# bkram/fmtuner-sdr

Hardware: AMD Instinct MI355X
Metric: IQ MS/s demodulated per GPU (2.4 MS/s FM channels, stereo+RDS) at 1/2/4/8 MI355X (higher is better)
Workload: dtype f32 (FIR operands f16 hi+lo, f32 accumulate)

## Files before the change

fmtuner-sdr_amd/csrc/fmx_kernels.hip:

```cpp
#include <hip/hip_ext.h>
#include <hip/hip_fp16.h>
#include <hip/hip_runtime.h>

#include <cstddef>
#include <type_traits>

#include "fmx_internal.h"
#include "fmx_math.h"
#include "fmx_synth.h"


namespace fmx {

#define FE_T 768
#define FE_HALO_IQ 120
#define AU_T 768
#define AU_HALO 120
#define AU_RHALO 32
#define AU_MAXOUT 256

static constexpr float kPiF = 3.14159265358979323846f;

#define FMX_CONST __attribute__((address_space(4)))
template <typename T> __device__ __forceinline__ const FMX_CONST T *cptr(const T *p) {
// ... 525 lines not shown
        fe_decimate<M, TPP>(inq, Q, D->dec_poly, tid, ai, aq);
        int myclip = 0;
#pragma unroll
        for (int r = 0; r < 3; ++r) {
          const int j = 3 * tid + r;
          if (j < cnt) {
            const float yr = ai[r] * D->dec_scale;
            const float yi = aq[r] * D->dec_scale;
            if (fabsf(yr) >= 0.995f || fabsf(yi) >= 0.995f) myclip++;
            xin[FE_HALO_IQ + j] = make_float2(yr, yi);
            if (a.bb_out) {
              float *o = a.bb_out + (size_t)c * a.bb_stride + 2 * (size_t)(n0 + j);
              o[0] = yr;
              o[1] = yi;
            }
          }
        }
        if (myclip) atomicAdd(&sh->clip, myclip);
        __syncthreads();
      }
    } else if (a.in_mode == FE_IN_CF) {
      int myclip = 0;
      for (int j = tid; j < cnt; j += 256) {
        const float *p = a.in_f + (size_t)c * a.in_stride + 2 * (size_t)(n0 + j);
        const float xr = p[0], xi = p[1];
        if (fabsf(xr) >= 0.995f || fabsf(xi) >= 0.995f) myclip++;
        xin[FE_HALO_IQ + j] = make_float2(xr, xi);
      }
      if (myclip) atomicAdd(&sh->clip, myclip);
    } else if (a.in_mode == FE_IN_U8_DIRECT) {
      int myclip = 0;
      const uint8_t *p = a.iq + (size_t)c * a.iq_stride;
      for (int j = tid; j < cnt; j += 256) {
        const uint8_t ib = p[2 * (size_t)(n0 + j)], qb = p[2 * (size_t)(n0 + j) + 1];
        if (ib == 0 || ib == 255 || qb == 0 || qb == 255) myclip++;
        if (want_sig) sig.sample(ib, qb);
        xin[FE_HALO_IQ + j] = make_float2(((float)ib - 127.0f) / 127.5f, ((float)qb - 127.0f) / 127.5f);
      }
      if (myclip) atomicAdd(&sh->clip, myclip);
    }
    __syncthreads();

    if (demod) {
      FE_STAMP(0)
      float A = 1.0f, BI = 0.0f, BQ = 0.0f;
      float2 xv[3];
#pragma unroll
      for (int r = 0; r < 3; ++r) {
        const int j = 3 * tid + r;
        xv[r] = (j < cnt) ? xin[FE_HALO_IQ + j] : make_float2(0.0f, 0.0f);
        if (j < cnt) {
          BI = xv[r].x + dc_c * BI;
          BQ = xv[r].y + dc_c * BQ;
          A = dc_c * A;
        }
      }
#pragma unroll
      for (int d = 1; d < 64; d <<= 1) {
        const float pA = __shfl_up(A, d);
        const float pI = __shfl_up(BI, d);
        const float pQ = __shfl_up(BQ, d);
        if (lane >= d) {
          BI = A * pI + BI;
          BQ = A * pQ + BQ;
          A = A * pA;
        }
      }
      if (lane == 63) {
        sh->wave_a[wave] = A;
        sh->wave_bi[wave] = BI;
        sh->wave_bq[wave] = BQ;
      }
      float eA = __shfl_up(A, 1), eI = __shfl_up(BI, 1), eQ = __shfl_up(BQ, 1);
      if (lane == 0) {
        eA = 1.0f;
        eI = 0.0f;
        eQ = 0.0f;
      }
      __syncthreads();
      float vI = sh->carry_i, vQ = sh->carry_q;
      for (int w = 0; w < wave; ++w) {
        vI = sh->wave_a[w] * vI + sh->wave_bi[w];
        vQ = sh->wave_a[w] * vQ + sh->wave_bq[w];
      }
      vI = eA * vI + eI;
      vQ = eA * vQ + eQ;
#pragma unroll
      for (int r = 0; r < 3; ++r) {
        const int j = 3 * tid + r;
        if (j < cnt) {
          const float tI = dc_a1 * vI;
          const float tQ = dc_a1 * vQ;
          const float nI = xv[r].x - tI;
          const float nQ = xv[r].y - tQ;
          xin[FE_HALO_IQ + j] = make_float2(nI - vI, nQ - vQ);
          vI = nI;
          vQ = nQ;
          if (j == cnt - 1) {
            sh->carry_i = nI;
            sh->carry_q = nQ;
          }
        }
      }
      __syncthreads();
      FE_STAMP(1)
      {
        float zr[3], zi[3];
        fir_c3(xin, FE_HALO_IQ + 3 * tid, iqh, iqL, zr, zi);
#pragma unroll
        for (int r = 0; r < 3; ++r) {
          const int j = 3 * tid + r;
          if (j < cnt) yb[1 + j] = make_float2(zr[r] * iqscale, zi[r] * iqscale);
        }
        if (tid == 0) yb[0] = make_float2(sh->fd_re, sh->fd_im);
      }
      __syncthreads();
      if (par.agc != 0) {
        if (tid == 0) {
          for (int j = 0; j < cnt; ++j) {
            const float2 x = yb[1 + j];
            const float yr = x.x * agc_g, yi = x.y * agc_g;
            const float y2 = yr * yr + yi * yi;
            agc_y2p = (float)((1.0 - (double)agc_bw) * (double)agc_y2p + (double)(agc_bw * y2));
            if (agc_y2p > 1e-6f) agc_g *= expf(-0.5f * agc_bw * logf(agc_y2p));
            if (agc_g > 1e6f) agc_g = 1e6f;
            yb[1 + j] = make_float2(yr, yi);
          }
        }
        __syncthreads();
      }
      FE_STAMP(2)
      const float ref = (par.fd_ref != 0.0f) ? par.fd_ref : D->fd_ref;
      for (int j = tid; j < cnt; j += 256) {
        const float2 p = yb[j], r = yb[1 + j];
        const float re = p.x * r.x + p.y * r.y;
        const float im = p.x * r.y - p.y * r.x;
        const float m = fmx_atan2f(im, re) * ref;
        mx[FMX_HIST + j] = m;
        if (rds) rb[32 + j] = m;
        if (a.mpx_out) a.mpx_out[(size_t)c * a.mpx_stride + n0 + j] = m;
      }
    } else if (a.in_mode == FE_IN_MPX) {
      for (int j = tid; j < cnt; j += 256) {
        const float m = a.in_f[(size_t)c * a.in_stride + n0 + j];
        mx[FMX_HIST + j] = m;
        if (rds) rb[32 + j] = m;
      }
    }
    __syncthreads();

    FE_STAMP(3)
    FmxSched en3[3];
    if (rds) {
#pragma unroll
      for (int k = 0; k < 3; ++k) {
        const int e = e_pos + tid + 256 * k;
        en3[k] = (e < sched_n) ? sched[e] : FmxSched{0xFFFF, 0.0f};
      }
    }
    if (pilot) {
      float z[3];
      fir_r3p(mx, FMX_HIST + 3 * tid, D->pilot_pad, D->pilot_pair, D->pilot_len, z);
#pragma unroll
      for (int r = 0; r < 3; ++r) {
        const int j = 3 * tid + r;
        if (j < cnt) a.pilot_out[(size_t)c * a.pilot_stride + n0 + j] = z[r];
      }
    }
    FE_STAMP(4)
    if (rds) {
      int last = -1;
#pragma unroll
      for (int k = 0; k < 3; ++k) {
        const int e = e_pos + tid + 256 * k;
        if (e < sched_n && (en3[k].packed & 0xFFFF) < n0 + cnt) {
          a.rds_out[(size_t)c * a.rds_stride + e] =
              resamp_out_pair<FMX_RDS_RS_SUB>(rsp, en3[k].packed, en3[k].mu, rb + 32 - n0);
          last = e;
        }
        __builtin_amdgcn_sched_barrier(0);
      }
      if (last >= 0) atomicMax(&sh->e_end, last + 1);
    }
    __syncthreads();
    if (rds) e_pos = sh->e_end;
    FE_STAMP(5)
    {
      float2 cx = make_float2(0.0f, 0.0f);
      float cm0 = 0.0f, cm1 = 0.0f;
      if (demod && tid < FE_HALO_IQ) cx = xin[tid + cnt];
      cm0 = mx[tid + cnt];
      cm1 = mx[tid + 256 + cnt];
      const float2 cy = yb[cnt];
      const float crb = (rds && tid < 32) ? rb[cnt + tid] : 0.0f;
      __syncthreads();
      if (rds && tid < 32) rb[tid] = crb;
      if (demod && tid < FE_HALO_IQ) xin[tid] = cx;
      mx[tid] = cm0;
      mx[tid + 256] = cm1;
      if (tid == 0 && demod) {
        sh->fd_re = cy.x;
        sh->fd_im = cy.y;
      }
      __syncthreads();
    }
  }

  if (a.in_mode == FE_IN_U8_DECIM && M > 1) {
    const long total = (long)n * M;
    uint16_t keep[2];
    int cntk = 0;
    for (int h = tid; h < L - 1; h += 256) {
      const long g = total - (L - 1) + h;
      uint16_t v;
      if (g >= 0) v = iq16(g);
      else {
        const int hh = (L - 1) + (int)g;
        v = (uint16_t)dhist[2 * hh] | ((uint16_t)dhist[2 * hh + 1] << 8);
      }
      keep[cntk++] = v;
    }
    __syncthreads();
    cntk = 0;
    uint8_t *dh = a.dec_hist + (size_t)c * 2 * FMX_MAX_DEC;
    for (int h = tid; h < L - 1; h += 256) {
      const uint16_t v = keep[cntk++];
      dh[2 * h] = (uint8_t)(v & 255);
      dh[2 * h + 1] = (uint8_t)(v >> 8);
    }
    if (tid == 0) {
      long nv = (long)dec_valid + total;
      a.dec_valid[c] = (int)(nv > (L - 1) ? (L - 1) : nv);
    }
  }
  if (demod) {
    for (int h = tid; h < FE_HALO_IQ; h += 256) {
      const float2 v = xin[h];
      a.iq_hist[(size_t)c * (FMX_IQ_MAXLEN - 1) + h] = float2_t{v.x, v.y};
    }
    if (tid == 0) {
      a.dc_v[2 * c] = sh->carry_i;
      a.dc_v[2 * c + 1] = sh->carry_q;
      a.fd_prev[2 * c] = sh->fd_re;
      a.fd_prev[2 * c + 1] = sh->fd_im;
      if (par.agc != 0) {
        a.agc[2 * c] = agc_g;
        a.agc[2 * c + 1] = agc_y2p;
      }
    }
  }
  if (hist_out) {
    float *hist = a.st_hist_wr + (size_t)c * FMX_HIST;
    for (int h = tid; h < FMX_HIST; h += 256) hist[h] = mx[h];
  }
  if (rds) {
    if (tid < 32) a.rds_hist[(size_t)c * 32 + tid] = rb[tid];
    if (tid == 0) a.rds_count[c] = sched_n;
  }
  FE_STAMP(6)
#ifdef FMX_STAMPS
  if (a.dbg && tid == 0)
    for (int k = 0; k < 8; ++k) atomicAdd(a.dbg + k, st_acc[k]);
#endif
#undef FE_STAMP
  if (tid == 0 && a.clip_out && a.in_mode != FE_IN_MPX)
    a.clip_out[c] = (n > 0) ? (float)sh->clip / (float)n : 0.0f;
  if (want_sig) fe_signal_sums(a, sig, sgp, c, lane, wave, tid);
}

__device__ __forceinline__ void dma_dword(const float *src, uint32_t lds) {
  unsigned keep;
  asm volatile("s_mov_b32 %0, m0\n\ts_mov_b32 m0, %2\n\ts_nop 0\n\tglobal_load_lds_dword %1, off\n\ts_mov_b32 m0, %0"
               : "=&s"(keep)
               : "v"(src), "s"(__builtin_amdgcn_readfirstlane(lds))
               : "memory");
}
__device__ __forceinline__ void dma_dword_s(const float *base, uint32_t voff, uint32_t lds) {
  __builtin_amdgcn_global_load_lds(reinterpret_cast<const char *>(base) + voff,
                                   (__attribute__((address_space(3))) void *)(uintptr_t)__builtin_amdgcn_readfirstlane(lds), 4, 0, 0);
}
__device__ __forceinline__ void dma_dwordx3(const float *src, uint32_t lds) {
  unsigned keep;
  asm volatile("s_mov_b32 %0, m0\n\ts_mov_b32 m0, %2\n\ts_nop 0\n\tglobal_load_lds_dwordx3 %1, off\n\ts_mov_b32 m0, %0"
               : "=&s"(keep)
               : "v"(src), "s"(__builtin_amdgcn_readfirstlane(lds))
               : "memory");
}
__device__ __forceinline__ uint32_t lds_addr(const void *p) {
  return __builtin_amdgcn_readfirstlane((uint32_t)(uintptr_t)(const __attribute__((address_space(3))) char *)p);
}
__device__ __forceinline__ void word_sincos(uint32_t theta, float *s, float *c) { fmx_word_sincos(theta, s, c); }

#include "fmx_pll.inc"

#define AU2_T 2048
#define AU2_PT 8
#define AU2_MAXOUT (AU2_T / 3 + 16)
#define AU_IMG (AU_HALO + AU2_T + 24)
#define AU_FN (AU_RHALO + AU2_T)
struct AuShared {
  float2 xf[AU_IMG > AU_FN ? AU_IMG : AU_FN] __attribute__((aligned(16)));
  float2 fh[AU_RHALO];
  float2 o[AU2_MAXOUT];
  float hT[FMX_AF_SUB][FMX_NPFB];
  float2 hf[AU_HALO];
  float ws[3][4][2];
  float iir[4];
  int eb, ee, count;
  uint32_t lrq[((2 * FMX_LR_QN + 63) / 64) * 64] __attribute__((aligned(16)));
};

template <int CTRL, int ROWS> __device__ __forceinline__ float dpp_or(float x, float id) {
  return __builtin_bit_cast(float, __builtin_amdgcn_update_dpp(__builtin_bit_cast(int, id), __builtin_bit_cast(int, x), CTRL,
                                                               ROWS, 0xF, false));
}
#define WAVE_AFF_STEP(CTRL, ROWS)                                                       \
  {                                                                                   \
    const float pA_ = dpp_or<CTRL, ROWS>(A, 1.0f), p1_ = dpp_or<CTRL, ROWS>(B1, 0.0f); \
    const float p2_ = dpp_or<CTRL, ROWS>(B2, 0.0f);                                     \
    B1 = A * p1_ + B1;                                                                \
    B2 = A * p2_ + B2;                                                                \
    A = A * pA_;                                                                      \
  }
__device__ __forceinline__ void wave_affine_scan(float &A, float &B1, float &B2) {
  WAVE_AFF_STEP(0x111, 0xF)
  WAVE_AFF_STEP(0x112, 0xF)
  WAVE_AFF_STEP(0x114, 0xF)
  WAVE_AFF_STEP(0x118, 0xF)
  WAVE_AFF_STEP(0x142, 0xA)
  WAVE_AFF_STEP(0x143, 0xC)
}
#undef WAVE_AFF_STEP
__device__ __forceinline__ void wave_affine_prev(float A, float B1, float B2, float &eA, float &e1, float &e2) {
  eA = dpp_or<0x138, 0xF>(A, 1.0f);
  e1 = dpp_or<0x138, 0xF>(B1, 0.0f);
  e2 = dpp_or<0x138, 0xF>(B2, 0.0f);
}

__device__ __forceinline__ void au_scan_prev(float A, float BL, float BR, float cl, float cr, float (*ws)[4][2],
                                             float &pl, float &pr) {
  const int tid = threadIdx.x, lane = tid & 63, wave = tid >> 6;
  wave_affine_scan(A, BL, BR);
  if (lane == 63) {
    ws[0][wave][0] = A;
    ws[1][wave][0] = BL;
    ws[2][wave][0] = BR;
  }
  float eA, eL, eR;
  wave_affine_prev(A, BL, BR, eA, eL, eR);
  __syncthreads();
  float vl = cl, vr = cr;
  for (int w = 0; w < wave; ++w) {
    vl = ws[0][w][0] * vl + ws[1][w][0];
    vr = ws[0][w][0] * vr + ws[2][w][0];
  }
  pl = eA * vl + eL;
  pr = eA * vr + eR;
  __syncthreads();
}

#ifndef FMX_AU_WPE
#define FMX_AU_WPE 1
#endif
__global__ __launch_bounds__(256) __attribute__((amdgpu_waves_per_eu(FMX_AU_WPE))) void k_audio(AudioArgs a) {
  extern __shared__ __align__(16) unsigned char au_smem[];
  AuShared &S = *reinterpret_cast<AuShared *>(au_smem);
  const int c = au_channel(blockIdx.x, a.C, a.in_tiled != 0);
  const int tid = threadIdx.x;
  const FmxDesign *__restrict__ D = a.des;
  const FmxChanParam par = a.par[c];
  const int n = a.n;
  const bool mono = (a.mode == 2 || a.mode == 3);
  const bool lrfir = (a.mode == 0 || a.mode == 4);
  const bool af = (a.mode != 4);
  const bool pipe_mono = (a.mode == 3);
  const int deemph = par.deemph;
  const float dalpha = (deemph == 0) ? D->deemph_alpha[0] : ((deemph == 1) ? D->deemph_alpha[1] : par.deemph_alpha);
  const bool de_on = deemph != 2;
  const float dc_alpha = mono ? 0.0008f : 0.005f;
  const float de_a1 = -(1.0f - dalpha);
  const float dc_a1 = -1.0f + dc_alpha;
  if (a.sig_out && blockIdx.x * 256 < (unsigned)a.C) {
    const int cs = blockIdx.x * 256 + tid;
    if (cs < a.C)
      signal_level_eval(a.sig_sums + 6 * (size_t)cs, a.sig_samples, a.sig_par + 4 * (size_t)cs,
                        a.sig_smooth + 2 * (size_t)cs, a.sig_out + cs);
  }
  float *lrh = a.lr_hist + (size_t)c * 2 * (FMX_LR_LEN - 1);
  float *win = mono ? a.mono_win + (size_t)c * 32 : a.af_win + (size_t)c * 2 * 32;
  float2 *const F = S.xf;
  float2 cx = make_float2(0.0f, 0.0f);
  if (lrfir && tid < AU_HALO) cx = make_float2(lrh[tid], lrh[(FMX_LR_LEN - 1) + tid]);
  if (af)
    for (int h = tid; h < AU_RHALO; h += 256) S.fh[h] = make_float2(win[h], mono ? 0.0f : win[32 + h]);
  float *iir = mono ? a.mono_iir + (size_t)c * 2 : a.af_iir + (size_t)c * 4;
  if (af && tid == 0) {
    if (mono) {
      S.iir[0] = iir[0];
      S.iir[1] = 0.0f;
      S.iir[2] = iir[1];
      S.iir[3] = 0.0f;
    } else {
      for (int k = 0; k < 4; ++k) S.iir[k] = iir[k];
    }
  }
  const FmxSched *sched = nullptr;
  int sched_n = 0;
  if (af) {
    const int g = a.group[c];
    sched = a.sched + (size_t)g * a.sched_stride;
    sched_n = a.sched_n[g];
    for (int k = tid; k < FMX_NPFB * FMX_AF_SUB; k += 256) {
      const int b = k / FMX_AF_SUB, nn = k % FMX_AF_SUB;
      S.hT[nn][b] = D->af_h[k];
    }
  }
  if (lrfir) {
    static_assert(FMX_LR_QN % 2 == 0, "dword window");
    const float *qs = reinterpret_cast<const float *>(&D->lr_q16[0][0][0]);
    for (int p = tid >> 6; p < (2 * FMX_LR_QN + 63) / 64; p += 4)
      dma_dword(qs + min(64 * p + (tid & 63), 2 * FMX_LR_QN - 1), lds_addr(&S.lrq[64 * p]));
  }
  if (tid == 0) {
    S.eb = 0;
    S.count = 0;
  }
  const bool tiled = a.in_tiled != 0;
  const float *inl = a.in_l + (tiled ? lr_tile_idx(c, 0, a.in_stride) : (size_t)c * a.in_stride);
  const float *inr = mono ? nullptr : a.in_r + (tiled ? lr_tile_idx(c, 0, a.in_stride) : (size_t)c * a.in_stride);
  auto ti = [&](int j) __attribute__((always_inline)) { return tiled ? (j >> 4) * 32 + (j & 15) : j; };
  const float sc = D->lr_scale;
  int mrem = 0, mtot = 0;
  if (a.mute) {
    mrem = a.mute[2 * c];
    mtot = a.mute[2 * c + 1];
  }
  const int mdone = (mtot > mrem) ? mtot - mrem : 0;
  const int mfade = max(1, min(a.mute_fade, mtot / 2));
  __syncthreads();
  for (int n0 = 0; n0 < n; n0 += AU2_T) {
    const int cnt = min(AU2_T, n - n0);
    FmxSched en3[3];
    if (af) {
      const int eb = S.eb;
#pragma unroll
      for (int k = 0; k < 3; ++k) {
        const int e = eb + tid + 256 * k;
        en3[k] = (e < sched_n) ? sched[e] : FmxSched{0xFFFF, 0.0f};
      }
    }
    {
      float vl[AU2_PT], vr[AU2_PT];
#pragma unroll
      for (int k = 0; k < AU2_PT; ++k) {
        const int j = tid + 256 * k;
        vl[k] = (j < cnt) ? inl[ti(n0 + j)] : 0.0f;
        vr[k] = (j < cnt && !mono) ? inr[ti(n0 + j)] : 0.0f;
      }
      if (lrfir) {
        _Float16 *im = reinterpret_cast<_Float16 *>(S.xf);
        auto put = [&](int i, float l, float r) __attribute__((always_inline)) {
          l *= 1024.0f;
          r *= 1024.0f;
          const _Float16 lh = (_Float16)l, rh = (_Float16)r;
          im[i] = lh;
          im[AU_IMG + i] = (_Float16)(l - (float)lh);
          im[2 * AU_IMG + i] = rh;
          im[3 * AU_IMG + i] = (_Float16)(r - (float)rh);
        };
        if (tid < AU_HALO) put(tid, cx.x, cx.y);
#pragma unroll
        for (int k = 0; k < AU2_PT; ++k) put(AU_HALO + tid + 256 * k, vl[k], vr[k]);
        if (tid < AU_IMG - AU_HALO - AU2_T) put(AU_HALO + AU2_T + tid, 0.0f, 0.0f);
#pragma unroll
        for (int k = 0; k < AU2_PT; ++k) {
          const int j = tid + 256 * k;
          if (j >= cnt - AU_HALO && j < cnt) S.hf[j - (cnt - AU_HALO)] = make_float2(vl[k], vr[k]);
        }
        if (tid < AU_HALO && tid >= cnt) S.hf[tid - cnt] = cx;
      } else {
#pragma unroll
        for (int k = 0; k < AU2_PT; ++k) {
          const int j = tid + 256 * k;
          if (j < cnt) F[AU_RHALO + j] = make_float2(vl[k], vr[k]);
        }
      }
      if (!lrfir && af && tid < AU_RHALO) F[tid] = S.fh[tid];
    }
    if (tid == 0) S.ee = S.eb;
    __syncthreads();
    if (lrfir) {
      typedef _Float16 f16x8_t __attribute__((ext_vector_type(8)));
      typedef float f32x4_t __attribute__((ext_vector_type(4)));
      typedef unsigned int u32x4 __attribute__((ext_vector_type(4)));
      const int lane = tid & 63, wave = tid >> 6, col = lane & 15, g = lane >> 4;
      const _Float16 *im = reinterpret_cast<const _Float16 *>(S.xf);
      const int xb = 16 * (32 * wave + col) + 8 * g;
      const f16x8_t *bLh = reinterpret_cast<const f16x8_t *>(im + xb);
      const f16x8_t *bLl = reinterpret_cast<const f16x8_t *>(im + AU_IMG + xb);
      const f16x8_t *bRh = reinterpret_cast<const f16x8_t *>(im + 2 * AU_IMG + xb);
      const f16x8_t *bRl = reinterpret_cast<const f16x8_t *>(im + 3 * AU_IMG + xb);
      const int qb = 8 * g + 15 - col, qc = qb & 1;
      const uint32_t *qh = &S.lrq[0] + qc * FMX_LR_QN + (qb - qc) / 2;
      const uint32_t *ql = qh + FMX_LR_QN / 2;
      auto frag = [&](int ks, const uint32_t *q) __attribute__((always_inline)) {
        return u32x4{q[16 * ks], q[16 * ks + 1], q[16 * ks + 2], q[16 * ks + 3]};
      };
      f32x4_t aL[2], aR[2];
      aL[0] = aL[1] = aR[0] = aR[1] = f32x4_t{0.0f, 0.0f, 0.0f, 0.0f};
      u32x4 ah = frag(0, qh), al = frag(0, ql);
#pragma unroll
      for (int ks = 0; ks < FMX_LR_KS; ++ks) {
        const f16x8_t ahi = __builtin_bit_cast(f16x8_t, ah), alo = __builtin_bit_cast(f16x8_t, al);
        if (ks + 1 < FMX_LR_KS) {
          ah = frag(ks + 1, qh);
          al = frag(ks + 1, ql);
        }
#pragma unroll
        for (int u = 0; u < 2; ++u) {
          const f16x8_t lh = bLh[32 * u + 4 * ks], ll = bLl[32 * u + 4 * ks];
          const f16x8_t rh = bRh[32 * u + 4 * ks], rl = bRl[32 * u + 4 * ks];
          aL[u] = __builtin_amdgcn_mfma_f32_16x16x32_f16(lh, ahi, aL[u], 0, 0, 0);
          aR[u] = __builtin_amdgcn_mfma_f32_16x16x32_f16(rh, ahi, aR[u], 0, 0, 0);
          aL[u] = __builtin_amdgcn_mfma_f32_16x16x32_f16(ll, ahi, aL[u], 0, 0, 0);
          aR[u] = __builtin_amdgcn_mfma_f32_16x16x32_f16(rl, ahi, aR[u], 0, 0, 0);
          aL[u] = __builtin_amdgcn_mfma_f32_16x16x32_f16(lh, alo, aL[u], 0, 0, 0);
          aR[u] = __builtin_amdgcn_mfma_f32_16x16x32_f16(rh, alo, aR[u], 0, 0, 0);
        }
      }
      if (tid < AU_HALO) cx = S.hf[tid];
      __syncthreads();
      if (af && tid < AU_RHALO) F[tid] = S.fh[tid];
      const float osc = sc * (1.0f / 4194304.0f);
#pragma unroll
      for (int u = 0; u < 2; ++u) {
#pragma unroll
        for (int i = 0; i < 4; ++i) {
          const int j = 256 * (2 * wave + u) + 16 * (4 * g + i) + col;
          const float2 y = make_float2(aL[u][i] * osc, aR[u][i] * osc);
          if (af) F[AU_RHALO + j] = y;
          if (a.lr_out_l && j < cnt) {
            a.lr_out_l[(size_t)c * a.lr_out_stride + n0 + j] = y.x;
            a.lr_out_r[(size_t)c * a.lr_out_stride + n0 + j] = y.y;
          }
        }
      }
    }
    __syncthreads();
    if (af) {
      const int eb = S.eb;
      int last = -1;
#pragma unroll
      for (int k = 0; k < 3; ++k) {
        const int e = eb + tid + 256 * k;
        if (e < sched_n && (en3[k].packed & 0xFFFF) < n0 + cnt) {
          const int i = (en3[k].packed & 0xFFFF) - n0;
          const int b = (en3[k].packed >> 16) & 0xFF;
          const bool boundary = (en3[k].packed >> 24) & 1;
          const int b0 = boundary ? FMX_NPFB - 1 : b, b1 = boundary ? 0 : b + 1;
          const int i0 = boundary ? i - 1 : i;
          float y0l = 0.0f, y0r = 0.0f, y1l = 0.0f, y1r = 0.0f;
          auto mac = [](float &y, float h, float x) __attribute__((always_inline)) {
            float t;
            asm("v_mul_f32 %0, %2, %3\n\tv_add_f32 %1, %1, %0" : "=&v"(t), "+v"(y) : "v"(h), "v"(x));
          };
#pragma unroll
          for (int m = 0; m < FMX_AF_SUB; ++m) {
            const float2 v0 = F[AU_RHALO + i0 - (FMX_AF_SUB - 1) + m];
            const float2 v1 = F[AU_RHALO + i - (FMX_AF_SUB - 1) + m];
            const float h0 = S.hT[FMX_AF_SUB - 1 - m][b0], h1 = S.hT[FMX_AF_SUB - 1 - m][b1];
            mac(y0l, h0, v0.x);
            mac(y0r, h0, v0.y);
            mac(y1l, h1, v1.x);
            mac(y1r, h1, v1.y);
          }
          const float mu = en3[k].mu, omu = 1.0f - mu;
          float yl, yr;
          asm("v_mul_f32 %0, %2, %3\n\tv_mul_f32 %1, %2, %4" : "=&v"(yl), "=&v"(yr) : "v"(omu), "v"(y0l), "v"(y0r));
          mac(yl, mu, y1l);
          mac(yr, mu, y1r);
          S.o[e - eb] = make_float2(yl, yr);
          last = e;
        }
      }
      if (last >= 0) atomicMax(&S.ee, last + 1);
      __syncthreads();
      const int m = S.ee - eb;
      float xl[3], xr[3];
      bool on[3];
#pragma unroll
      for (int k = 0; k < 3; ++k) {
        const int q = 3 * tid + k;
        on[k] = q < m;
        const float2 v = on[k] ? S.o[q] : make_float2(0.0f, 0.0f);
        xl[k] = v.x;
        xr[k] = v.y;
      }
      auto compose = [&](float a_, const float *bl, const float *br, float &A, float &BL, float &BR) {
        A = 1.0f;
        BL = 0.0f;
        BR = 0.0f;
#pragma unroll
        for (int k = 0; k < 3; ++k)
          if (on[k]) {
            BL = a_ * BL + bl[k];
            BR = a_ * BR + br[k];
            A = a_ * A;
          }
      };
      if (de_on) {
        float A, BL, BR, pl, pr;
        compose(-de_a1, xl, xr, A, BL, BR);
        au_scan_prev(A, BL, BR, S.iir[0], S.iir[1], S.ws, pl, pr);
#pragma unroll
        for (int k = 0; k < 3; ++k)
          if (on[k]) {
            const float vl = xl[k] - de_a1 * pl, vr = xr[k] - de_a1 * pr;
            if (3 * tid + k == m - 1) {
              S.iir[0] = vl;
              S.iir[1] = vr;
            }
            pl = vl;
            pr = vr;
            xl[k] = dalpha * vl;
            xr[k] = dalpha * vr;
          }
      }
      float A, BL, BR, ql, qr;
      compose(-dc_a1, xl, xr, A, BL, BR);
      au_scan_prev(A, BL, BR, S.iir[2], S.iir[3], S.ws, ql, qr);
      const int o0 = S.count;
#pragma unroll
      for (int k = 0; k < 3; ++k)
        if (on[k]) {
          const float vl = xl[k] - dc_a1 * ql, vr = xr[k] - dc_a1 * qr;
          float yl = vl - ql, yr = vr - qr;
          if (3 * tid + k == m - 1) {
            S.iir[2] = vl;
            S.iir[3] = vr;
          }
          ql = vl;
          qr = vr;
          if (pipe_mono) yl = yl * 0.5f;
          if (a.clamp) {
            yl = d_clamp(yl, -1.0f, 1.0f);
            yr = d_clamp(yr, -1.0f, 1.0f);
          }
          const int o = o0 + 3 * tid + k;
          if (o < mrem) {
            const int idx = mdone + o;
            float gain = 0.0f;
            if (idx < mfade) gain = 1.0f - ((float)idx / (float)mfade);
            else if (idx >= mtot - mfade) gain = (float)(mtot - idx) / (float)mfade;
            gain = d_clamp(gain, 0.0f, 1.0f);
            yl *= gain;
            yr *= gain;
          }
          if (o < a.cap) {
            a.out_l[(size_t)c * a.out_stride + o] = yl;
            if (pipe_mono) a.out_r[(size_t)c * a.out_stride + o] = yl;
            else if (!mono) a.out_r[(size_t)c * a.out_stride + o] = yr;
          }
        }
      __syncthreads();
      if (tid == 0) {
        S.count = o0 + m;
        S.eb = eb + m;
      }
    }
    {
      float2 cf = make_float2(0.0f, 0.0f);
      if (af && tid < AU_RHALO) cf = F[tid + cnt];
      __syncthreads();
      if (af && tid < AU_RHALO) S.fh[tid] = cf;
      __syncthreads();
    }
  }
  if (lrfir && tid < AU_HALO) {
    lrh[tid] = cx.x;
    lrh[(FMX_LR_LEN - 1) + tid] = cx.y;
  }
  if (af) {
    for (int h = tid; h < AU_RHALO; h += 256) {
      const float2 v = S.fh[h];
      win[h] = v.x;
      if (!mono) win[32 + h] = v.y;
    }
    if (tid == 0) {
      if (mono) {
        iir[0] = S.iir[0];
        iir[1] = S.iir[2];
      } else {
        for (int k = 0; k < 4; ++k) iir[k] = S.iir[k];
      }
    }
    const int nout = S.count < a.cap ? S.count : a.cap;
    if (tid == 0 && a.out_count) a.out_count[c] = nout;
    if (tid == 0 && a.mute && mrem > 0 && nout > 0) {
      const int mc = min(nout, mrem);
      a.mute[2 * c] = mrem - mc;
      if (mrem - mc == 0) a.mute[2 * c + 1] = 0;
    }
  }
}

enum { OA = 0, OB = 1, OC = 2, OCP = 3, OD = 4, OINV = 5 };
__device__ __forceinline__ int bs_block_number(int off) {
  return (off == OA) ? 0 : (off == OB) ? 1 : (off == OC || off == OCP) ? 2 : (off == OD) ? 3 : 0;
}
__device__ __forceinline__ int bs_next(int off) {
  return (off == OA) ? OB : (off == OB) ? OC : (off == OC || off == OCP) ? OD : OA;
}
__device__ __forceinline__ int bs_offset_for(uint32_t s) {
  switch (s) {
    case 0x3D8: return OA;
    case 0x3D4: return OB;
    case 0x25C: return OC;
    case 0x3CC: return OCP;
    case 0x258: return OD;
    default: return OINV;
  }
}
__constant__ uint32_t c_parity[26] = {0x200, 0x100, 0x080, 0x040, 0x020, 0x010, 0x008, 0x004, 0x002,
                                      0x001, 0x2DC, 0x16E, 0x0B7, 0x287, 0x39F, 0x313, 0x355, 0x376,
                                      0x1BB, 0x201, 0x3DC, 0x1EE, 0x0F7, 0x2A7, 0x38F, 0x31B};
__device__ __forceinline__ uint32_t bs_syndrome(uint32_t v) {
  uint32_t r = 0;
#pragma unroll
  for (int k = 0; k < 26; ++k) r ^= ((v >> k) & 1u) ? c_parity[25 - k] : 0u;
  return r;
}
__device__ __forceinline__ bool pulse_follows(uint32_t pos, int off, uint32_t opos, int ooff) {
  const uint32_t d = pos - opos;
  return d % 26 == 0 && d / 26 <= 6 && off != OINV && ooff != OINV &&
         ((uint32_t)bs_block_number(ooff) + d / 26) % 4 == (uint32_t)bs_block_number(off);
}

#define RDS_LPC 8
#define RDS_CPW (64 / RDS_LPC)
#define RDS_SYMQ 12
#ifndef RDS_PF
#define RDS_PF 3
#endif
#ifndef RDS_NR
#define RDS_NR 4
#endif
static_assert(RDS_PF < RDS_NR && (RDS_NR & (RDS_NR - 1)) == 0 && 3 * RDS_PF <= 63, "k_rds input ring");
static_assert(FMX_RDS_DECIM == 3 * RDS_LPC, "three samples per lane and decimation period");
struct RdsBits {
  float bi_prev_re, bi_prev_im, bi_even, bi_odd;
  uint32_t bi_clock, bi_polarity;
  int delta_prev;
  uint32_t bs_bitcount, bs_until_next, bs_reg, bs_err_mask_lo, bs_err_mask_hi;
  int bs_expected, bs_in_sync, bs_err_ptr;
  uint32_t bs_pulse_pos[4];
  int bs_pulse_off[4];
  uint32_t bs_blk_raw[4];
  uint16_t bs_blk_data[4];
  uint8_t bs_blk_flags[4];
  uint32_t bs_bits_since_lost;
};
struct RdsCold {
  RdsBits s;
  uint32_t pad_[(sizeof(RdsBits) / 4) % 2 == 0 ? 1 : 2];
};
static_assert((sizeof(RdsCold) / 4) % 2 == 1, "RdsCold must have an odd dword stride");
__device__ __forceinline__ void rds_bits_load(RdsBits &b, const FmxRdsState &g) {
  b.bi_prev_re = g.bi_prev_re;
  b.bi_prev_im = g.bi_prev_im;
  b.bi_even = g.bi_even;
  b.bi_odd = g.bi_odd;
  b.bi_clock = g.bi_clock;
  b.bi_polarity = g.bi_polarity;
  b.delta_prev = g.delta_prev;
  b.bs_bitcount = g.bs_bitcount;
  b.bs_until_next = g.bs_until_next;
  b.bs_reg = g.bs_reg;
  b.bs_err_mask_lo = g.bs_err_mask_lo;
  b.bs_err_mask_hi = g.bs_err_mask_hi;
  b.bs_expected = g.bs_expected;
  b.bs_in_sync = g.bs_in_sync;
  b.bs_err_ptr = g.bs_err_ptr;
  for (int i = 0; i < 4; ++i) {
    b.bs_pulse_pos[i] = g.bs_pulse_pos[i];
    b.bs_pulse_off[i] = g.bs_pulse_off[i];
    b.bs_blk_raw[i] = g.bs_blk_raw[i];
    b.bs_blk_data[i] = g.bs_blk_data[i];
    b.bs_blk_flags[i] = g.bs_blk_flags[i];
  }
  b.bs_bits_since_lost = g.bs_bits_since_lost;
}
__device__ __forceinline__ void rds_bits_store(FmxRdsState &g, const RdsBits &b) {
  g.bi_prev_re = b.bi_prev_re;
  g.bi_prev_im = b.bi_prev_im;
  g.bi_even = b.bi_even;
  g.bi_odd = b.bi_odd;
  g.bi_clock = b.bi_clock;
  g.bi_polarity = b.bi_polarity;
  g.delta_prev = b.delta_prev;
  g.bs_bitcount = b.bs_bitcount;
  g.bs_until_next = b.bs_until_next;
  g.bs_reg = b.bs_reg;
  g.bs_err_mask_lo = b.bs_err_mask_lo;
  g.bs_err_mask_hi = b.bs_err_mask_hi;
  g.bs_expected = b.bs_expected;
  g.bs_in_sync = b.bs_in_sync;
  g.bs_err_ptr = b.bs_err_ptr;
  for (int i = 0; i < 4; ++i) {
    g.bs_pulse_pos[i] = b.bs_pulse_pos[i];
    g.bs_pulse_off[i] = b.bs_pulse_off[i];
    g.bs_blk_raw[i] = b.bs_blk_raw[i];
    g.bs_blk_data[i] = b.bs_blk_data[i];
    g.bs_blk_flags[i] = b.bs_blk_flags[i];
  }
  g.bs_bits_since_lost = b.bs_bits_since_lost;
}
#define RS_KS 16
#define RS_XP 80
#define RS_XS 20
typedef float rs_f32x4 __attribute__((ext_vector_type(4)));
__device__ __forceinline__ int rs_k0_of(uint32_t p0) {
  const int i0 = p0 & 0xFFFF;
  return ((((p0 >> 24) & 1) ? i0 - 1 : i0) - (FMX_RDS_RS_SUB - 1)) & ~3;
}
__device__ __forceinline__ int rs_tile_k0(const FmxSched &e) {
  return rs_k0_of(__builtin_amdgcn_readlane(e.packed, 0));
}
__device__ __forceinline__ void rs_load_w(const float *mrow, const float *wrow, bool lcv, int n, int lq, int k0,
                                          float4 (&v)[4]) {
#pragma unroll
  for (int j = 0; j < 4; ++j) {
    const int k = k0 + 16 * lq + 4 * j;
    const bool ok = k < (lcv ? n : INT_MIN);
    const float *base = (ok && k < 0) ? wrow : mrow;
    v[j] = *reinterpret_cast<const float4 *>(base + (ok ? k : 0));
  }
}
__device__ __forceinline__ void rs_store_w(float *xrow, bool lcv, int n, int lq, int k0, const float4 (&v)[4]) {
  float4 w[4];
#pragma unroll
  for (int j = 0; j < 4; ++j) {
    const bool ok = k0 + 16 * lq + 4 * j < (lcv ? n : INT_MIN);
    w[j] = ok ? v[j] : make_float4(0.0f, 0.0f, 0.0f, 0.0f);
  }
  *reinterpret_cast<float4 *>(&xrow[4 * lq]) = make_float4(w[0].x, w[1].x, w[2].x, w[3].x);
  *reinterpret_cast<float4 *>(&xrow[RS_XS + 4 * lq]) = make_float4(w[0].y, w[1].y, w[2].y, w[3].y);
  *reinterpret_cast<float4 *>(&xrow[2 * RS_XS + 4 * lq]) = make_float4(w[0].z, w[1].z, w[2].z, w[3].z);
  *reinterpret_cast<float4 *>(&xrow[3 * RS_XS + 4 * lq]) = make_float4(w[0].w, w[1].w, w[2].w, w[3].w);
}
__device__ __forceinline__ int rs_tile_build(const float (*tab)[FMX_RDS_RS_SUB + 1], const FmxSched &en, int kk,
                                             float (&hv)[RS_KS]) {
  const int i = en.packed & 0xFFFF, b = (en.packed >> 16) & 0xFF;
  const bool bnd = (en.packed >> 24) & 1;
  const int s_r = (bnd ? i - 1 : i) - (FMX_RDS_RS_SUB - 1);
  const int row0 = bnd ? FMX_NPFB - 1 : b, row1 = bnd ? FMX_NPFB : ((b + 1) & (FMX_NPFB - 1));
  const int k0 = rs_tile_k0(en);
  const int m0 = k0 + kk - s_r;
  const uint32_t p15 = __builtin_amdgcn_readlane(en.packed, 15);
  const int i15 = p15 & 0xFFFF;
  const int s15 = ((((p15 >> 24) & 1) ? i15 - 1 : i15) - (FMX_RDS_RS_SUB - 1));
  const int ks = min(RS_KS, (s15 + FMX_RDS_RS_SUB - k0 + 3) / 4);
  const float mu = en.mu, mu1 = 1.0f - mu;
#pragma unroll
  for (int st = 0; st < RS_KS; ++st) {
    const int m = m0 + 4 * st;
    const int mc = min(max(m, 0), FMX_RDS_RS_SUB);
    const bool in = m >= 0 && m <= FMX_RDS_RS_SUB;
    hv[st] = in ? mu1 * tab[row0][mc] + mu * tab[row1][mc] : 0.0f;
  }
  return ks;
}
__device__ __forceinline__ rs_f32x4 rs_tile_mma(const float *xrow, const float (&hv)[RS_KS], int ks, int kk) {
  float xv[RS_KS];
#pragma unroll
  for (int q = 0; q < RS_KS / 4; ++q) {
    const float4 x4 = *reinterpret_cast<const float4 *>(&xrow[RS_XS * kk + 4 * q]);
    xv[4 * q] = x4.x;
// ... 1763 lines not shown
```

Before: 324,800.

## Vectorize audio input loads and f16 image stores, streamline resampler taps

In the LR-FIR path each thread now handles 8 contiguous samples, loading them as float4 when the pointers are 16-byte aligned and writing the hi/lo f16 split as 16-byte vector LDS stores instead of scalar halves. The polyphase resampler's filter table gains a wrapped extra column so both tap rows come from one base pointer. The two sample windows are merged into one sliding load with a boundary select, roughly halving the LDS reads per output. The contiguous per-thread mapping changes which threads write the halo buffer and adds an alignment-dependent branch.

```diff
diff --git a/fmtuner-sdr_amd/csrc/fmx_kernels.hip b/fmtuner-sdr_amd/csrc/fmx_kernels.hip
--- a/fmtuner-sdr_amd/csrc/fmx_kernels.hip
+++ b/fmtuner-sdr_amd/csrc/fmx_kernels.hip
@@ -851,7 +851,7 @@
   float2 xf[AU_IMG > AU_FN ? AU_IMG : AU_FN] __attribute__((aligned(16)));
   float2 fh[AU_RHALO];
   float2 o[AU2_MAXOUT];
-  float hT[FMX_AF_SUB][FMX_NPFB];
+  float hT[FMX_AF_SUB][FMX_NPFB + 1];
   float2 hf[AU_HALO];
   float ws[3][4][2];
   float iir[4];
@@ -908,6 +908,7 @@
   __syncthreads();
 }
 
+typedef _Float16 au_f16x8_t __attribute__((ext_vector_type(8)));
 #ifndef FMX_AU_WPE
 #define FMX_AU_WPE 1
 #endif
@@ -961,7 +962,9 @@
     sched_n = a.sched_n[g];
     for (int k = tid; k < FMX_NPFB * FMX_AF_SUB; k += 256) {
       const int b = k / FMX_AF_SUB, nn = k % FMX_AF_SUB;
-      S.hT[nn][b] = D->af_h[k];
+      const float h = D->af_h[k];
+      S.hT[nn][b] = h;
+      if (b == 0) S.hT[nn][FMX_NPFB] = h;
     }
   }
   if (lrfir) {
@@ -978,6 +981,7 @@
   const float *inl = a.in_l + (tiled ? lr_tile_idx(c, 0, a.in_stride) : (size_t)c * a.in_stride);
   const float *inr = mono ? nullptr : a.in_r + (tiled ? lr_tile_idx(c, 0, a.in_stride) : (size_t)c * a.in_stride);
   auto ti = [&](int j) __attribute__((always_inline)) { return tiled ? (j >> 4) * 32 + (j & 15) : j; };
+  const bool in16 = lrfir && ((reinterpret_cast<uintptr_t>(inl) | reinterpret_cast<uintptr_t>(inr)) & 15) == 0;
   const float sc = D->lr_scale;
   int mrem = 0, mtot = 0;
   if (a.mute) {
@@ -1000,34 +1004,62 @@
     }
     {
       float vl[AU2_PT], vr[AU2_PT];
-#pragma unroll
-      for (int k = 0; k < AU2_PT; ++k) {
-        const int j = tid + 256 * k;
-        vl[k] = (j < cnt) ? inl[ti(n0 + j)] : 0.0f;
-        vr[k] = (j < cnt && !mono) ? inr[ti(n0 + j)] : 0.0f;
-      }
       if (lrfir) {
+        const int j0 = AU2_PT * tid;
+        const float *pl = inl + ti(n0 + j0), *pr = inr + ti(n0 + j0);
+        if (in16 && j0 + AU2_PT <= cnt) {
+          const float4 l0 = *reinterpret_cast<const float4 *>(pl), l1 = *reinterpret_cast<const float4 *>(pl + 4);
+          const float4 r0 = *reinterpret_cast<const float4 *>(pr), r1 = *reinterpret_cast<const float4 *>(pr + 4);
+          vl[0] = l0.x, vl[1] = l0.y, vl[2] = l0.z, vl[3] = l0.w, vl[4] = l1.x, vl[5] = l1.y, vl[6] = l1.z, vl[7] = l1.w;
+          vr[0] = r0.x, vr[1] = r0.y, vr[2] = r0.z, vr[3] = r0.w, vr[4] = r1.x, vr[5] = r1.y, vr[6] = r1.z, vr[7] = r1.w;
+        } else {
+#pragma unroll
+          for (int k = 0; k < AU2_PT; ++k) {
+            vl[k] = (j0 + k < cnt) ? pl[k] : 0.0f;
+            vr[k] = (j0 + k < cnt) ? pr[k] : 0.0f;
+          }
+        }
         _Float16 *im = reinterpret_cast<_Float16 *>(S.xf);
+        auto split = [](float x, _Float16 &hi, _Float16 &lo) __attribute__((always_inline)) {
+          x *= 1024.0f;
+          hi = (_Float16)x;
+          lo = (_Float16)(x - (float)hi);
+        };
         auto put = [&](int i, float l, float r) __attribute__((always_inline)) {
-          l *= 1024.0f;
-          r *= 1024.0f;
-          const _Float16 lh = (_Float16)l, rh = (_Float16)r;
-          im[i] = lh;
-          im[AU_IMG + i] = (_Float16)(l - (float)lh);
-          im[2 * AU_IMG + i] = rh;
-          im[3 * AU_IMG + i] = (_Float16)(r - (float)rh);
+          split(l, im[i], im[AU_IMG + i]);
+          split(r, im[2 * AU_IMG + i], im[3 * AU_IMG + i]);
         };
         if (tid < AU_HALO) put(tid, cx.x, cx.y);
-#pragma unroll
-        for (int k = 0; k < AU2_PT; ++k) put(AU_HALO + tid + 256 * k, vl[k], vr[k]);
+        static_assert((AU_HALO * 2) % 16 == 0 && (AU_IMG * 2) % 16 == 0 && AU2_PT == 8, "16-byte image writes");
+        au_f16x8_t lh, ll, rh, rl;
+#pragma unroll
+        for (int k = 0; k < AU2_PT; ++k) {
+          _Float16 h, l;
+          split(vl[k], h, l);
+          lh[k] = h, ll[k] = l;
+          split(vr[k], h, l);
+          rh[k] = h, rl[k] = l;
+        }
+        *reinterpret_cast<au_f16x8_t *>(im + AU_HALO + j0) = lh;
+        *reinterpret_cast<au_f16x8_t *>(im + AU_IMG + AU_HALO + j0) = ll;
+        *reinterpret_cast<au_f16x8_t *>(im + 2 * AU_IMG + AU_HALO + j0) = rh;
+        *reinterpret_cast<au_f16x8_t *>(im + 3 * AU_IMG + AU_HALO + j0) = rl;
         if (tid < AU_IMG - AU_HALO - AU2_T) put(AU_HALO + AU2_T + tid, 0.0f, 0.0f);
+        if (j0 + AU2_PT > cnt - AU_HALO && j0 < cnt) {
+#pragma unroll
+          for (int k = 0; k < AU2_PT; ++k) {
+            const int j = j0 + k;
+            if (j >= cnt - AU_HALO && j < cnt) S.hf[j - (cnt - AU_HALO)] = make_float2(vl[k], vr[k]);
+          }
+        }
+        if (tid < AU_HALO && tid >= cnt) S.hf[tid - cnt] = cx;
+      } else {
 #pragma unroll
         for (int k = 0; k < AU2_PT; ++k) {
           const int j = tid + 256 * k;
-          if (j >= cnt - AU_HALO && j < cnt) S.hf[j - (cnt - AU_HALO)] = make_float2(vl[k], vr[k]);
-        }
-        if (tid < AU_HALO && tid >= cnt) S.hf[tid - cnt] = cx;
-      } else {
+          vl[k] = (j < cnt) ? inl[ti(n0 + j)] : 0.0f;
+          vr[k] = (j < cnt && !mono) ? inr[ti(n0 + j)] : 0.0f;
+        }
 #pragma unroll
         for (int k = 0; k < AU2_PT; ++k) {
           const int j = tid + 256 * k;
@@ -1106,22 +1138,25 @@
           const int i = (en3[k].packed & 0xFFFF) - n0;
           const int b = (en3[k].packed >> 16) & 0xFF;
           const bool boundary = (en3[k].packed >> 24) & 1;
-          const int b0 = boundary ? FMX_NPFB - 1 : b, b1 = boundary ? 0 : b + 1;
-          const int i0 = boundary ? i - 1 : i;
+          const int b0 = boundary ? FMX_NPFB - 1 : b;
+          const float2 *w = F + AU_RHALO + i - FMX_AF_SUB;
+          const float *hp = &S.hT[0][b0];
           float y0l = 0.0f, y0r = 0.0f, y1l = 0.0f, y1r = 0.0f;
           auto mac = [](float &y, float h, float x) __attribute__((always_inline)) {
             float t;
             asm("v_mul_f32 %0, %2, %3\n\tv_add_f32 %1, %1, %0" : "=&v"(t), "+v"(y) : "v"(h), "v"(x));
           };
+          float2 prev = w[0];
 #pragma unroll
           for (int m = 0; m < FMX_AF_SUB; ++m) {
-            const float2 v0 = F[AU_RHALO + i0 - (FMX_AF_SUB - 1) + m];
-            const float2 v1 = F[AU_RHALO + i - (FMX_AF_SUB - 1) + m];
-            const float h0 = S.hT[FMX_AF_SUB - 1 - m][b0], h1 = S.hT[FMX_AF_SUB - 1 - m][b1];
+            const float2 v1 = w[m + 1];
+            const float2 v0 = make_float2(boundary ? prev.x : v1.x, boundary ? prev.y : v1.y);
+            const float h0 = hp[(FMX_AF_SUB - 1 - m) * (FMX_NPFB + 1)], h1 = hp[(FMX_AF_SUB - 1 - m) * (FMX_NPFB + 1) + 1];
             mac(y0l, h0, v0.x);
             mac(y0r, h0, v0.y);
             mac(y1l, h1, v1.x);
             mac(y1r, h1, v1.y);
+            prev = v1;
           }
           const float mu = en3[k].mu, omu = 1.0f - mu;
           float yl, yr;
```

Measured after the change: 324,500. Within noise of the previous version (-0.1%).
